# TinyMPC/TinyMPC

Hardware: AMD Instinct MI355X
Metric: QP solves/sec (+ ADMM iters/sec), 64k-batch quadrotor hover (higher is better)
Workload: dtype f64; 1 GPU; quadrotor_hovering (nx=12, nu=4, N=10), 65536 identical instances per GPU, closed-loop MPC steps from a cold start (BASELINE configs[1]); batch_per_gpu=65536, total_batch=65536, parallelism=batch-sharded x1, mpc_steps_per_launch=8, stats_exchange=none (one rank), launcher=plain process

## Files before the change

### tinympc_amd/csrc/admm_kernel.hip.h

```cpp
#pragma once
#include <hip/hip_runtime.h>
#include <stdint.h>

namespace tinympc_amd {

enum : int {
    TAB_MB = 0,
    TAB_MF1 = 256,
    TAB_MF2 = 512,
    TAB_PT = 768,
    TAB_VEC = 1024,
    TAB_BOUNDS = 1024 + 16 * 16,
};
enum : int {
    VEC_CB = 0,
    VEC_CF = 1,
    VEC_QR = 2,
    VEC_SMASK = 3,
    VEC_NIM = 4,
    VEC_SOCFLAG = 5,
    VEC_CONE_BASE = 6,
    VEC_CONE_MU = 7,
    VEC_LINFLAG = 9,
    VEC_TLINFLAG = 10,
// ... 549 lines not shown
    return __builtin_nontemporal_load(p);
#else
    return *p;
#endif
}
__device__ __forceinline__ void store_primal(double* p, double v) {
#if TINYMPC_PRIM_STORE == 1
    __builtin_nontemporal_store(v, p);
#elif TINYMPC_PRIM_STORE == 2
    asm volatile("global_store_dwordx2 %0, %1, off sc1" : : "v"(p), "v"(v) : "memory");
#elif TINYMPC_PRIM_STORE == 3
    asm volatile("global_store_dwordx2 %0, %1, off sc0 sc1" : : "v"(p), "v"(v) : "memory");
#elif TINYMPC_PRIM_STORE == 4
    asm volatile("global_store_dwordx2 %0, %1, off sc0 sc1 nt" : : "v"(p), "v"(v) : "memory");
#else
    *p = v;
#endif
}

__device__ __forceinline__ double grp_max16(double v) {
#pragma unroll
    for (int off = 8; off >= 1; off >>= 1) v = fmax(v, __shfl_xor(v, off, 16));
    return v;
}
template <int W>
__device__ __forceinline__ double grp_maxw(double v) {
#pragma unroll
    for (int off = W / 2; off >= 1; off >>= 1) v = fmax(v, __shfl_xor(v, off, W));
    return v;
}

__device__ __forceinline__ double soc_component(double s0, double s1, double s2, double mine, int c, float mu) {
#pragma clang fp contract(off)
    const double u0 = s2 * (double)mu;
    const double q0 = s0 * s0, q1 = s1 * s1;
    const double q = q0 + q1;
    const bool sure_inside = (u0 > 1e-30) && (q <= (u0 * u0) * (1.0 - 0x1p-20)) && (q < 1e70);
    if (__builtin_amdgcn_ballot_w64(!sure_inside) == 0ull) return mine;
    const float a = (float)sqrt(q);
    const double ad = (double)a;
    const bool below = ad <= -u0, inside = ad <= u0;
    const bool outside = !below && !inside && (ad >= fabs(u0));
    double r = (below || !inside) ? 0.0 : mine;
    if (__builtin_amdgcn_ballot_w64(outside) != 0ull) {
        const double scale = 0.5 * (1.0 + u0 / ad);
        const double last = (double)(a / mu);
        const double o = scale * ((c == 2) ? last : mine);
        r = outside ? o : r;
    }
    return r;
}

__device__ __forceinline__ bool soc_all_inside(double s0, double s1, double s2, float mu) {
#pragma clang fp contract(off)
    const double u0 = s2 * (double)mu;
    const double q0 = s0 * s0, q1 = s1 * s1;
    const double q = q0 + q1;
    const bool sure_inside = (u0 > 1e-30) & (u0 < 1e300) & (q <= (u0 * u0) * (1.0 - 0x1p-20)) & (q < 1e70);
    return __builtin_amdgcn_ballot_w64(!sure_inside) == 0ull;
}
__device__ __forceinline__ void soc_project3(double s0, double s1, double s2, float mu, float rmu, bool rmu_exact, double& r0, double& r1, double& r2) {
#pragma clang fp contract(off)
    const double u0 = s2 * (double)mu;
    const double q0 = s0 * s0, q1 = s1 * s1;
    const double q = q0 + q1;
    const float a = (float)sqrt(q);
    const double ad = (double)a;
    const bool below = ad <= -u0, inside = ad <= u0;
    const bool outside = !below && !inside && (ad >= fabs(u0));
    const bool zero = below || !inside;
    r0 = zero ? 0.0 : s0; r1 = zero ? 0.0 : s1; r2 = zero ? 0.0 : s2;
    if (__builtin_amdgcn_ballot_w64(outside) != 0ull) {
        const double scale = 0.5 * (1.0 + u0 / ad);
        const double last = (double)(rmu_exact ? a * rmu : a / mu);
        r0 = outside ? scale * s0 : r0;
        r1 = outside ? scale * s1 : r1;
        r2 = outside ? scale * last : r2;
    }
}
__device__ __forceinline__ int soc_items_of(unsigned heads, int nx, int n) {
    int c = 0;
    for (unsigned m = heads; m; m &= m - 1) c += (__builtin_ctz(m) < nx) ? n : n - 1;
    return c;
}
constexpr int soc_item_passes(int nx, int nu, int n) { return ((nx / 3) * n + (nu / 3) * (n - 1) + 15) / 16; }

constexpr int ADAPT_LOG = 32;
__device__ __forceinline__ double taylor_step(double a, double d, double b) {
#pragma clang fp contract(off)
    const double t = d * b;
    return a + t;
}

constexpr int solve_kernel_waves_per_simd(int nz, int n, bool soc, bool lin = false, bool adapt = false) {
    if (lin) return 1;
    if (adapt) return n <= 10 ? 2 : 1;
    return (n <= 10 || 2 * ((soc ? 8 : 6) * n + 2 * nz + 8) + 40 <= 256) ? 2 : 1;
}

#ifndef TINYMPC_LIN_WAVES
#define TINYMPC_LIN_WAVES 0
#endif
constexpr long solve_kernel_lin_lds(int nx, int nu, int n, bool soc, int lin, int kmax, bool ub) {
    const int nz = nx + nu, csl = (nz + 1) | 1, cs = (nz + 1) | 1;
    return 8L * (nx * 16 + (ub ? 2 : 2 * n * 16) + ((lin & 1) ? 3 * kmax * 16 + 2 * 4 * n * csl : 0) +
                 ((lin & 2) ? 3 * n * kmax * 16 + 2 * 4 * n * csl : 0) + (soc ? (4 * n + 1) * 3 * cs : 0));
}
constexpr bool solve_kernel_lin_planes(int nx, int nu, int n, bool soc, int lin, int kmax, bool ub) {
    return lin != 0 && solve_kernel_lin_lds(nx, nu, n, soc, lin, kmax, ub) <= 64 * 1024 - 512;
}
constexpr int solve_kernel_lin_waves(int nx, int nu, int n, bool soc, int lin, int kmax, bool ub) {
    if (!solve_kernel_lin_planes(nx, nu, n, soc, lin, kmax, ub)) return 1;
    if (TINYMPC_LIN_WAVES > 0) return TINYMPC_LIN_WAVES;
    return (solve_kernel_waves_per_simd(nx + nu, n, soc) == 2 && 8 * solve_kernel_lin_lds(nx, nu, n, soc, lin, kmax, ub) <= 158 * 1024) ? 2 : 1;
}
template <int NF, int KMAX_, int LW_, int LPI_>
__device__ __forceinline__ void project_halfspace_columns(const int t, const int inst, const int n, const int csl, const int R0, const int S0,
                                                          double* pv, double* pg, const double* tab, const int tab_stride, const int nk) {
#pragma clang fp contract(off)
    for (int c = S0 + t; c < n; c += LPI_) {
        const int at = (inst * n + c) * csl + R0;
        const double* tk = tab + c * tab_stride;
        double z[NF], t0[NF];
#pragma unroll
        for (int r = 0; r < NF; ++r) { z[r] = pv[at + r]; t0[r] = z[r]; }
        for (int k = 0; k < nk; ++k) {
            double cv = 0.0;
#pragma unroll
            for (int r = 0; r < NF; ++r) { const double pr = tk[k * LW_ + R0 + r] * z[r]; cv = cv + pr; }
            const double bk = tk[KMAX_ * LW_ + k * LW_ + R0];
            if (cv > bk) {
                const double dist = (cv - bk) / tk[2 * KMAX_ * LW_ + k * LW_ + R0];
#pragma unroll
                for (int r = 0; r < NF; ++r) { const double pr = dist * tk[k * LW_ + R0 + r]; z[r] = z[r] - pr; }
            }
        }
#pragma unroll
        for (int r = 0; r < NF; ++r) { pv[at + r] = z[r]; pg[at + r] = t0[r] - z[r]; }
    }
}

template <int NX, int NU, int N, bool SOC, bool DBG, int MODE, int LIN = 0, bool HET = false, int KMAX = LIN_KMAX, bool ADAPT = false, bool UB = false, bool HALF = false,
          bool PF = false>
__global__ __launch_bounds__(64)
__attribute__((amdgpu_waves_per_eu(LIN != 0 ? solve_kernel_lin_waves(NX, NU, N, SOC, LIN, KMAX, UB) : solve_kernel_waves_per_simd(NX + NU, N, SOC, false, ADAPT),
                                   LIN != 0 ? solve_kernel_lin_waves(NX, NU, N, SOC, LIN, KMAX, UB) : solve_kernel_waves_per_simd(NX + NU, N, SOC, false, ADAPT))))
void admm_solve_kernel(const SolveArgs P) {
    constexpr bool LS = (LIN & 1) != 0, LT = (LIN & 2) != 0;
    constexpr int NZ = NX + NU;
    static_assert(NZ <= 16, "one instance per 16-lane DPP row");
    constexpr bool FUSED = MODE == 2 && LIN == 0 && fused_shape(NX, NU);
    static_assert(!HALF || (NZ <= 8 && FUSED && !SOC && !DBG && !HET && !ADAPT), "half rows: nx+nu <= 8, the plain box kernel on its fused step blocks");
    static_assert(!PF || (MODE == 2 && !SOC && !DBG && LIN == 0 && !HET && !ADAPT), "prefetch form: the plain box kernel");
    constexpr int RL = HALF ? 8 : 16;
    constexpr int IPW = 64 / RL;
    constexpr int RECD = N * NZ;
    constexpr int PF_PIECES = (IPW * RECD * 8 + 1023) / 1024;
    constexpr int PF_ARR = PF_PIECES * 128;
    constexpr unsigned long long RMASK = HALF ? 0xFFull : 0xFFFFull;
    const int lane = threadIdx.x & 63;
    const int j = lane & (RL - 1);
    const int grp = lane / RL;
    const bool is_state = j < NX;
    const bool is_input = (j >= NX) && (j < NZ);

    __shared__ double sPt[NX * 16];
    __shared__ double sLo[UB ? 1 : N * 16];
    __shared__ double sHi[UB ? 1 : N * 16];
    __shared__ double sLin[LS ? 3 * KMAX * 16 : 1];
    __shared__ double sTLin[LT ? 3 * N * KMAX * 16 : 1];
#ifndef TINYMPC_SOC_PD
#define TINYMPC_SOC_PD 2
#endif
    constexpr int SPD = TINYMPC_SOC_PD, SPR = SPD + 1;
    constexpr int CS = SOC ? ((NZ + 1) | 1) : 1;
    constexpr int SLOT_D = 3 * CS;
    constexpr int PL_GC = CS, PL_VC = 2 * CS;
    __shared__ double sC[SOC ? (4 * N + 1) * SLOT_D : 1];
    __shared__ double sP[ADAPT ? 4 * NX * NX : 1];
    constexpr int AKC = NX > NU ? NX : NU;
    __shared__ double sTab[ADAPT ? 3 * 16 * AKC : 1];
    __shared__ double sDl[ADAPT ? 4 * ADAPT_LOG : 1];
    if constexpr (ADAPT)
        for (int e = lane; e < 3 * 16 * AKC; e += 64) {
            const int t = e / (16 * AKC), r = e % (16 * AKC);
            sTab[e] = P.atab[t * 256 + (r % AKC) * 16 + r / AKC];
        }
    if constexpr (LS) for (int e = lane; e < 3 * KMAX * 16; e += 64) sLin[e] = P.tab[TAB_BOUNDS + 2 * N * 16 + e];
    if constexpr (LT) for (int e = lane; e < 3 * N * KMAX * 16; e += 64) sTLin[e] = P.tab[TAB_BOUNDS + 2 * N * 16 + 3 * KMAX * 16 + e];
    for (int e = lane; e < NX * 16; e += 64) sPt[e] = P.tab[TAB_PT + e];
    for (int e = lane; e < N * 16; e += 64) {
        if constexpr (!UB) {
            sLo[e] = P.tab[TAB_BOUNDS + e];
            sHi[e] = P.tab[TAB_BOUNDS + N * 16 + e];
        }
    }
    double mb[NZ], mf1[NX], mf2[NU];
#pragma unroll
    for (int k = 0; k < NZ; ++k) mb[k] = P.tab[TAB_MB + k * 16 + j];
#pragma unroll
    for (int k = 0; k < NX; ++k) mf1[k] = P.tab[TAB_MF1 + k * 16 + j];
#pragma unroll
    for (int k = 0; k < NU; ++k) mf2[k] = P.tab[TAB_MF2 + (NX + k) * 16 + j];
    double cb = P.tab[TAB_VEC + VEC_CB * 16 + j];
    double cf = P.tab[TAB_VEC + VEC_CF * 16 + j];
    double qr = P.tab[TAB_VEC + VEC_QR * 16 + j];
    const double smask = P.tab[TAB_VEC + VEC_SMASK * 16 + j];
    const double nim = P.tab[TAB_VEC + VEC_NIM * 16 + j];
    bool soc_lane = false, proj_lane = false;
    int cone_base = -1, cone_c = 0;
    double socmask = 0.0;
    if constexpr (SOC) {
        socmask = P.tab[TAB_VEC + VEC_SOCFLAG * 16 + j];
        soc_lane = socmask != 0.0;
        cone_base = (int)P.tab[TAB_VEC + VEC_CONE_BASE * 16 + j];
        cone_c = (cone_base >= 0) ? (j - cone_base) : 0;
        proj_lane = soc_lane && cone_base >= 0;
    }
    constexpr int SOC_PASSES = SOC ? (soc_item_passes(NX, NU, N) > 0 ? soc_item_passes(NX, NU, N) : 1) : 1;
    int item_at[SOC_PASSES];
    float item_mu[SOC_PASSES], item_rmu[SOC_PASSES];
    bool mu_pow2 = true;
    int soc_passes = 0;
    if constexpr (SOC) {
        if (lane < 3) {
            sC[4 * N * SLOT_D + lane] = lane == 2 ? 1.0 : 0.0;
            sC[4 * N * SLOT_D + PL_GC + lane] = 0.0;
            sC[4 * N * SLOT_D + PL_VC + lane] = lane == 2 ? 1.0 : 0.0;
        }
        const unsigned heads = (unsigned)(__builtin_amdgcn_ballot_w64(proj_lane && cone_c == 0) & 0xFFFFull);
#pragma unroll
        for (int p = 0; p < SOC_PASSES; ++p) {
            int t = p * 16 + j;
            item_at[p] = 4 * N * SLOT_D; item_mu[p] = 1.0f;
            if (heads && p * 16 < soc_items_of(heads, NX, N)) soc_passes = p + 1;
            for (unsigned m = heads; m; m &= m - 1) {
                const int hb = __builtin_ctz(m);
                const int cnt = hb < NX ? N : N - 1;
                if (t >= 0 && t < cnt) {
                    item_at[p] = (grp * N + t + (hb < NX ? 0 : 1)) * SLOT_D + hb;
                    item_mu[p] = (float)P.tab[TAB_VEC + VEC_CONE_MU * 16 + hb];
                    t = -1;
                } else if (t >= 0) t -= cnt;
            }
            item_rmu[p] = 1.0f / item_mu[p];
            const unsigned mb_ = __float_as_uint(item_mu[p]);
            const bool p2 = (mb_ & 0x807FFFFFu) == 0u && (mb_ >> 23) >= 127u - 60u && (mb_ >> 23) <= 127u + 60u;
            if (__builtin_amdgcn_ballot_w64(!p2) != 0ull) mu_pow2 = false;
        }
    }
    bool lin_lane = false, tlin_lane = false;
    if constexpr (LS) lin_lane = P.tab[TAB_VEC + VEC_LINFLAG * 16 + j] != 0.0;
    if constexpr (LT) tlin_lane = P.tab[TAB_VEC + VEC_TLINFLAG * 16 + j] != 0.0;
    constexpr bool LPL = solve_kernel_lin_planes(NX, NU, N, SOC, LIN, KMAX, UB);
    constexpr bool LSP = LS && LPL, LTP = LT && LPL, LSR = LS && !LPL, LTR = LT && !LPL;
    constexpr int CSL = LPL ? ((NZ + 1) | 1) : 1;
    __shared__ double sLV[LSP ? 4 * N * CSL : 1], sLG[LSP ? 4 * N * CSL : 1];
    __shared__ double sTV[LTP ? 4 * N * CSL : 1], sTG[LTP ? 4 * N * CSL : 1];
    double ones[(LSR || LTR) ? 16 : 1];
#pragma unroll
    for (int k = 0; k < ((LSR || LTR) ? 16 : 1); ++k) ones[k] = 1.0;
    bool lin_x_on = false, lin_u_on = false, tlin_x_on = false, tlin_u_on = false;
    if constexpr (LS) { lin_x_on = P.tab[TAB_VEC + VEC_LINFLAG * 16] != 0.0; lin_u_on = P.tab[TAB_VEC + VEC_LINFLAG * 16 + NX] != 0.0; }
    if constexpr (LT) { tlin_x_on = P.tab[TAB_VEC + VEC_TLINFLAG * 16] != 0.0; tlin_u_on = P.tab[TAB_VEC + VEC_TLINFLAG * 16 + NX] != 0.0; }
    double rho = P.rho;
    __builtin_amdgcn_fence(__ATOMIC_RELEASE, "wavefront");
    __builtin_amdgcn_wave_barrier();

    const double lo_u = P.tab[TAB_BOUNDS + (N > 1 ? 16 : 0) + j], hi_u = P.tab[TAB_BOUNDS + N * 16 + (N > 1 ? 16 : 0) + j];
    const double lo_u0 = P.tab[TAB_BOUNDS + j], hi_u0 = P.tab[TAB_BOUNDS + N * 16 + j];
    const int ninst = PF ? P.batch : (P.index ? *P.count : (P.perm ? P.perm_count : P.batch));
    const int ntiles = (ninst + IPW - 1) / IPW;
    const bool resumed = !PF && P.index != nullptr;
    const bool has_traj = !PF && P.traj != nullptr;
    extern __shared__ __attribute__((aligned(16))) double sPF[];
    typedef const __attribute__((address_space(1))) void* pf_gptr;
    typedef __attribute__((address_space(3))) void* pf_lptr;
    constexpr int PF_S0 = 128, PF_S1 = PF_S0 + PF_ARR, PF_S2 = PF_S1 + PF_ARR, PF_S3 = PF_S2 + PF_ARR;
    auto pf_issue = [&](const int t) {
        const int tl = P.reverse ? ntiles - 1 - t : t;
        __builtin_amdgcn_global_load_lds((pf_gptr)(P.x0 + ((size_t)tl * (IPW * NX) + (size_t)lane * 2)), (pf_lptr)sPF, 16, 0, 0);
        const size_t t0 = (size_t)tl * (IPW * RECD) + (size_t)lane * 2;
        auto arr = [&](const double* p, const int at) {
#pragma unroll
            for (int q = 0; q < PF_PIECES; ++q) __builtin_amdgcn_global_load_lds((pf_gptr)(p + t0 + q * 128), (pf_lptr)(sPF + at + q * 128), 16, 0, 0);
        };
        if (!P.cold) { arr(P.slack, PF_S0); arr(P.dual, PF_S1); arr(P.slack_prev, PF_S2); }
        if (P.pf_mask & 8) arr(P.ref, P.cold ? PF_S0 : PF_S3);
    };
    unsigned pf_ticket = 0u;
    const int pf_shard = PF ? (int)(blockIdx.x % (unsigned)(P.pf_shards > 0 ? P.pf_shards : 1)) : 0;
    typedef __attribute__((address_space(1))) unsigned* pf_ctr_t;
    unsigned long long pf_ctr_bits = PF ? (unsigned long long)(P.pf_counter + 16 * pf_shard) : 0ull;
    if constexpr (PF) asm volatile("" : "+v"(pf_ctr_bits));
    const pf_ctr_t pf_ctr = (pf_ctr_t)pf_ctr_bits;
    auto pf_draw = [&]() { return lane == 0 ? __hip_atomic_fetch_add(pf_ctr, 1u, __ATOMIC_RELAXED, __HIP_MEMORY_SCOPE_AGENT) : 0u; };
    const unsigned pf_base = PF ? P.pf_base[pf_shard] : 0u;
    int pf_next = 0, pf_i = 0;
    bool pf_first = true;
    double* const sQX = sPF + PF_S3;
    if constexpr (PF) {
        if ((int)blockIdx.x < ntiles) {
            pf_issue((int)blockIdx.x);
            if (P.pf_static <= 1) pf_ticket = pf_draw();
        }
        if (P.ref_shared) {
            double rl = 0.0, qxs[N];
#pragma unroll
            for (int s = 0; s < N; ++s) {
                const bool valid = is_state || (is_input && s >= 1);
                const double r = valid ? P.ref[j - (is_input ? NZ : 0) + s * NZ] : 0.0;
                qxs[s] = -(r * qr);
                if (s == N - 1) rl = r;
            }
            double pt[NX];
#pragma unroll
            for (int k = 0; k < NX; ++k) pt[k] = sPt[k * 16 + j];
            double xp = 0.0;
            if constexpr (HALF) ring1_half<0, NX>(xp, rl, pt);
// ... 37 lines not shown
                for (int s = 0; s < N; ++s) {
                    const bool valid = is_state || (is_input && s >= 1);
                    const double r = valid ? sPF[at + lrow + s * NZ] : 0.0;
                    pfQXs[s] = -(r * qr);
                    if (s == N - 1) pf_rl = r;
                }
            };
            if (m & 8) { if (warm_t) own_ref(PF_S3); else own_ref(PF_S0); }
            else {
#pragma unroll
                for (int s = 0; s < N; ++s) pfQXs[s] = sQX[s * 16 + j];
            }
            if (warm_t) {
#pragma unroll
                for (int s = 0; s < N; ++s) pfVP[s] = sPF[PF_S2 + lrow + s * NZ];
            }
            asm volatile("s_waitcnt lgkmcnt(0)" ::: "memory");
            if (pf_next < ntiles) {
                if (pf_i + 2 >= P.pf_static) {
                    asm volatile("" ::: "memory");
                    pf_ticket = pf_draw();
                }
                pf_issue(pf_next);
            }
            ++pf_i;
        }
        (void)pfVN; (void)pfG; (void)pfVP; (void)pf_rl; (void)pf_x0; (void)pfQXs; (void)pf_first; (void)pf_ticket; (void)sQX; (void)pf_ctr; (void)pf_base; (void)pf_draw; (void)pf_i;
        if (slot < ninst) {
            const int b = PF ? slot : (resumed ? P.index[slot] : (P.perm ? P.perm[slot] : slot));
            const double* het = nullptr;
            if constexpr (HET) {
                het = P.het_tabs + (size_t)b * TAB_BOUNDS;
#pragma unroll
                for (int k = 0; k < NZ; ++k) mb[k] = het[TAB_MB + k * 16 + j];
#pragma unroll
                for (int k = 0; k < NX; ++k) mf1[k] = het[TAB_MF1 + k * 16 + j];
#pragma unroll
                for (int k = 0; k < NU; ++k) mf2[k] = het[TAB_MF2 + (NX + k) * 16 + j];
                cb = het[TAB_VEC + VEC_CB * 16 + j];
                cf = het[TAB_VEC + VEC_CF * 16 + j];
                qr = het[TAB_VEC + VEC_QR * 16 + j];
                rho = het[TAB_VEC + 8 * 16 + j];
            }
            if constexpr (ADAPT) {
                rho = P.arho[b];
                const double* aK = P.aK + (size_t)b * (NU * NX);
                if (is_state) {
#pragma unroll
                    for (int k = 0; k < NU; ++k) mb[NX + k] = -aK[k + NU * j];
#pragma unroll
                    for (int k = 0; k < NX; ++k) sP[grp * NX * NX + k + NX * j] = P.aP[(size_t)b * (NX * NX) + k + NX * j];
                } else if (is_input) {
#pragma unroll
                    for (int k = 0; k < NX; ++k) mf1[k] = -aK[(j - NX) + NU * k];
                }
                __builtin_amdgcn_fence(__ATOMIC_RELEASE, "wavefront");
                __builtin_amdgcn_wave_barrier();
            }
            const size_t lbase = (size_t)b * (N * NZ) + j - (is_input ? NZ : 0);
            double X[N], G[N], VN[N], VP[N], QX[N], Dn[N - 1];
            const int cw = grp * N * SLOT_D + (j < NZ ? j : NZ);
            const double x0v_in = is_state ? (PF ? pf_x0 : P.x0[(size_t)b * NX + j]) : 0.0;
            const int cl = grp * N * CSL + (j < NZ ? j : NZ);
            double VL[LSR ? N : 1], GL[LSR ? N : 1], VT[LTR ? N : 1], GT[LTR ? N : 1];
            double Qd[DBG ? N : 1], Pd[DBG ? N : 1], Dd[DBG ? N : 1];
            double ref_last = 0.0, qx_last_plain = 0.0;
#pragma unroll
            for (int s = 0; s < N; ++s) {
                const bool valid = is_state || (is_input && s >= 1);
                const size_t off = lbase + s * NZ;
                const bool warm = valid && !P.cold;
                if constexpr (PF) {
                    VN[s] = warm ? pfVN[s] : 0.0;
                    G[s] = warm ? pfG[s] : 0.0;
                    VP[s] = warm ? pfVP[s] : 0.0;
                    QX[s] = pfQXs[s];
                    X[s] = 0.0;
                    if (s == N - 1) ref_last = pf_rl;
                    continue;
                }
                const double r = valid ? (P.ref_shared ? P.ref[off - (size_t)b * (N * NZ)] : load_ref(P.ref + off)) : 0.0;
                VN[s] = warm ? P.slack[off] : 0.0;
                G[s] = warm ? P.dual[off] : 0.0;
                VP[s] = warm ? P.slack_prev[off] : 0.0;
                QX[s] = -(r * qr);
                X[s] = 0.0;
                if (s == N - 1) ref_last = r;
                if constexpr (SOC) {
                    double vc0 = (warm && soc_lane) ? (resumed ? P.cslack : P.prim)[off] : 0.0;
                    const double gc0 = (warm && soc_lane) ? P.cdual[off] : 0.0;
                    if (s == 0 && is_state && soc_lane && !resumed) vc0 = x0v_in;
                    sC[cw + s * SLOT_D] = vc0 - gc0;
                    sC[cw + s * SLOT_D + PL_GC] = gc0;
                    sC[cw + s * SLOT_D + PL_VC] = vc0;
                }
                if constexpr (LS) {
                    const double vl0 = (warm && lin_lane) ? (resumed ? P.lslack : P.prim)[off] : 0.0;
                    const double gl0 = (warm && lin_lane) ? P.ldual[off] : 0.0;
                    if constexpr (LSP) { sLV[cl + s * CSL] = vl0; sLG[cl + s * CSL] = gl0; } else { VL[s] = vl0; GL[s] = gl0; }
                }
                if constexpr (LT) {
                    const double vt0 = (warm && tlin_lane) ? (resumed ? P.tlslack : P.prim)[off] : 0.0;
                    const double gt0 = (warm && tlin_lane) ? P.tldual[off] : 0.0;
                    if constexpr (LTP) { sTV[cl + s * CSL] = vt0; sTG[cl + s * CSL] = gt0; } else { VT[s] = vt0; GT[s] = gt0; }
                }
                if constexpr (DBG) { Qd[s] = 0.0; Pd[s] = 0.0; Dd[s] = 0.0; }
            }
            double x0v = x0v_in;
            auto terminal_term = [&]() {
                double pt[NX];
#pragma unroll
                for (int k = 0; k < NX; ++k)
                    pt[k] = ADAPT ? sP[grp * NX * NX + k + NX * (is_state ? j : 0)] : (HET ? het[TAB_PT + k * 16 + j] : sPt[k * 16 + j]);
                double xp = 0.0;
                if constexpr (HALF) ring1_half<0, NX>(xp, ref_last, pt);
                else xp = ring_sum<MODE, 0, NX>(0.0, ref_last, pt);
                qx_last_plain = QX[N - 1];
                QX[N - 1] = is_state ? -xp : QX[N - 1];
            };
            int ndl = 0;
            auto flush_c = [&](int n) {
                __builtin_amdgcn_fence(__ATOMIC_RELEASE, "wavefront");
                __builtin_amdgcn_wave_barrier();
                if (P.aC2 && is_state) {
                    double* c2 = P.aC2 + (size_t)b * (NX * NX) + NX * j;
                    double v[NX], d[NX];
#pragma unroll
                    for (int k = 0; k < NX; ++k) { v[k] = c2[k]; d[k] = P.atab[ATAB_DC2 + k * 16 + j]; }
                    for (int i = 0; i < n; ++i) {
                        const double dl = sDl[grp * ADAPT_LOG + i];
#pragma unroll
                        for (int k = 0; k < NX; ++k) v[k] = taylor_step(v[k], dl, d[k]);
                    }
#pragma unroll
                    for (int k = 0; k < NX; ++k) c2[k] = v[k];
                }
                if (P.aC1 && j < NU) {
                    double* c1 = P.aC1 + (size_t)b * (NU * NU) + NU * j;
                    double v[NU], d[NU];
#pragma unroll
                    for (int k = 0; k < NU; ++k) { v[k] = c1[k]; d[k] = P.atab[ATAB_DC1 + k * 16 + j]; }
                    for (int i = 0; i < n; ++i) {
                        const double dl = sDl[grp * ADAPT_LOG + i];
#pragma unroll
                        for (int k = 0; k < NU; ++k) v[k] = taylor_step(v[k], dl, d[k]);
                    }
#pragma unroll
                    for (int k = 0; k < NU; ++k) c1[k] = v[k];
                }
            };
            if (!has_traj && !(PF && P.ref_shared)) terminal_term();
            const int traj_k0 = has_traj ? (P.traj_step0 + (P.traj_offsets ? P.traj_offsets[b] : 0)) : 0;

            int iter = 0, solved = 0, checked = 0;
            unsigned acc_iter = 0, acc_solved = 0;
            bool vp_touched = false;
            double rp = 0.0, rd = 0.0;
            const int nsteps = PF ? 1 : (P.steps > 1 ? P.steps : 1);
            const int iter_first = resumed ? P.iter_base : 0;
            for (int step = 0; step < nsteps; ++step) {
                X[0] = x0v;
                if (has_traj) {
                    if (is_state) {
#pragma unroll
                        for (int s = 0; s < N; ++s) {
                            int kk = traj_k0 + step + s;
                            kk = kk < P.traj_points ? kk : P.traj_points - 1;
                            const double r = P.traj[(size_t)kk * NX + j];
                            QX[s] = -(r * qr);
                            if (s == N - 1) ref_last = r;
                        }
                    }
                    terminal_term();
                }
                if (P.reset_duals) {
#pragma unroll
                    for (int s = 0; s < N; ++s) G[s] = 0.0;
                }
                if constexpr (SOC) {
                    if (step > 0) {
#pragma unroll
                        for (int s = 0; s < N; ++s) {
                            const double vc0 = soc_lane ? X[s] : 0.0;
                            sC[cw + s * SLOT_D] = vc0 - sC[cw + s * SLOT_D + PL_GC];
                            sC[cw + s * SLOT_D + PL_VC] = vc0;
                        }
                    }
                }
                if constexpr (LS) {
                    if (step > 0) {
#pragma unroll
                        for (int s = 0; s < N; ++s) { if constexpr (LSP) sLV[cl + s * CSL] = lin_lane ? X[s] : 0.0; else VL[s] = lin_lane ? X[s] : 0.0; }
                    } else if (is_state && lin_lane && !resumed) { if constexpr (LSP) sLV[cl] = x0v; else VL[0] = x0v; }
                }
                if constexpr (LT) {
                    if (step > 0) {
#pragma unroll
                        for (int s = 0; s < N; ++s) { if constexpr (LTP) sTV[cl + s * CSL] = tlin_lane ? X[s] : 0.0; else VT[s] = tlin_lane ? X[s] : 0.0; }
                    } else if (is_state && tlin_lane && !resumed) { if constexpr (LTP) sTV[cl] = x0v; else VT[0] = x0v; }
                }
                if constexpr (LPL) __builtin_amdgcn_fence(__ATOMIC_RELEASE, "wavefront");
                const int iter0 = iter_first;
                iter = iter0; solved = 0;
                if (resumed && P.check_termination > 0) checked = 1;
                int countdown = P.check_termination;
                double wr[SOC ? SPR : 1];
                bool gcz[SOC_PASSES];
#pragma unroll
                for (int p = 0; p < SOC_PASSES; ++p) gcz[p] = false;
                if constexpr (SOC) {
#pragma unroll
                    for (int d = 1; d <= SPR && d <= N; ++d) wr[(N - d) % SPR] = sC[cw + (N - d) * SLOT_D];
                }
                for (int it = iter0; it < P.max_iter; ++it) {
                    double lvr[LSP ? SPR : 1], lgr[LSP ? SPR : 1], tvr[LTP ? SPR : 1], tgr[LTP ? SPR : 1];
                    if constexpr (LPL) {
#pragma unroll
                        for (int d = 1; d <= SPR && d <= N; ++d) {
                            if constexpr (LSP) { lvr[(N - d) % SPR] = sLV[cl + (N - d) * CSL]; lgr[(N - d) % SPR] = sLG[cl + (N - d) * CSL]; }
                            if constexpr (LTP) { tvr[(N - d) % SPR] = sTV[cl + (N - d) * CSL]; tgr[(N - d) % SPR] = sTG[cl + (N - d) * CSL]; }
                        }
                    }
                    auto lin_w = [&](const int s_) { if constexpr (LSP) return lvr[s_ % SPR] - lgr[s_ % SPR]; else return VL[LSR ? s_ : 0] - GL[LSR ? s_ : 0]; };
                    auto tlin_w = [&](const int s_) { if constexpr (LTP) return tvr[s_ % SPR] - tgr[s_ % SPR]; else return VT[LTR ? s_ : 0] - GT[LTR ? s_ : 0]; };
                    double qhi;
                    {
                        double t = fma(-rho, VN[N - 1] - G[N - 1], QX[N - 1]);
                        if constexpr (SOC) t = fma(-rho, wr[(N - 1) % SPR], t);
                        if constexpr (LS) t = fma(-rho, lin_w(N - 1), t);
                        if constexpr (LT) t = fma(-rho, tlin_w(N - 1), t);
                        qhi = t;
                        if constexpr (DBG) {
                            double ql = fma(-rho, VN[N - 1] - G[N - 1], qx_last_plain);
                            if constexpr (SOC) ql = fma(-rho, wr[(N - 1) % SPR], ql);
                            if constexpr (LS) ql = fma(-rho, lin_w(N - 1), ql);
                            if constexpr (LT) ql = fma(-rho, tlin_w(N - 1), ql);
                            Qd[N - 1] = is_state ? ql : t;
                            Pd[N - 1] = t;
                        }
                    }
                    double pcur = qhi;
                    if constexpr (HALF) {
                        double tmpv = VN[N - 2] - G[N - 2];
#pragma unroll
                        for (int i = N - 2; i >= 0; --i) {
                            double qlo, res, dnp, tmpn;
                            constexpr int dummy = 0;
                            const int in = i > 0 ? i - 1 : dummy;
                            fused_backward_step_half<NX, NU>(qlo, res, dnp, tmpn, tmpv, VN[in], G[in], QX[i], rho, smask, cb, nim, cf, pcur, qhi, mb, mb + NX);
                            if (i + 1 <= N - 2) Dn[i + 1] = dnp;
                            tmpv = tmpn;
                            pcur = res;
                            qhi = qlo;
                        }
                        Dn[0] = fma(pcur, nim, cf);
                    }
#pragma unroll
                    for (int i = N - 2; i >= 0 && !HALF; --i) {
                        if constexpr (SOC) {
                            if (i >= SPD) wr[(i - SPD) % SPR] = sC[cw + (i - SPD) * SLOT_D];
                        }
                        if constexpr (LSP) { if (i >= SPD) { lvr[(i - SPD) % SPR] = sLV[cl + (i - SPD) * CSL]; lgr[(i - SPD) % SPR] = sLG[cl + (i - SPD) * CSL]; } }
                        if constexpr (LTP) { if (i >= SPD) { tvr[(i - SPD) % SPR] = sTV[cl + (i - SPD) * CSL]; tgr[(i - SPD) % SPR] = sTG[cl + (i - SPD) * CSL]; } }
                        if constexpr (SOC || LPL) __builtin_amdgcn_sched_barrier(0);
                        if constexpr (FUSED) {
                            double qlo, res;
                            if constexpr (SOC) fused_backward_step_soc<NX, NU>(qlo, res, VN[i], G[i], QX[i], wr[i % SPR], rho, smask, cb, pcur, qhi, mb, mb + NX);
                            else fused_backward_step<NX, NU>(qlo, res, VN[i], G[i], QX[i], rho, smask, cb, pcur, qhi, mb, mb + NX);
                            pcur = res;
                            Dn[i] = fma(res, nim, cf);
                            if constexpr (DBG) { Qd[i] = qlo; Pd[i] = res; Dd[i + 1] = res; }
                            qhi = qlo;
                            continue;
                        }
                        double qlo = fma(-rho, VN[i] - G[i], QX[i]);
                        if constexpr (SOC) qlo = fma(-rho, wr[i % SPR], qlo);
                        if constexpr (LS) qlo = fma(-rho, lin_w(i), qlo);
                        if constexpr (LT) qlo = fma(-rho, tlin_w(i), qlo);
                        const double res = ring_sum2<MODE, NX, NU>(fma(qlo, smask, cb), pcur, mb, qhi, mb + NX);
                        pcur = res;
                        Dn[i] = fma(res, nim, cf);
                        if constexpr (DBG) { Qd[i] = qlo; Pd[i] = res; Dd[i + 1] = res; }
                        qhi = qlo;
                    }
                    constexpr bool LAZY_RES = N <= 12;
                    constexpr bool TIGHT = FUSED && !HALF && LAZY_RES && !SOC && NX % 4 == 0;
                    double pmax = 0.0, dmax = 0.0;
                    auto slot_update = [&](const int s, const double lo, const double hi, const double gcv, const double glv, const double gtv) {
                        const double xi = X[s];
                        const double t = xi + G[s];
                        const double vn = TIGHT ? vclamp64(lo, hi, t) : vmin64(hi, vmax64(lo, t));
                        if constexpr (!LAZY_RES) {
                            pmax = resid_max<true>(pmax, xi - vn);
                            dmax = resid_max<true>(dmax, VP[s] - vn);
                        }
                        G[s] = t - vn;
                        VN[s] = vn;
                        if constexpr (SOC) {
                            sC[cw + s * SLOT_D] = fma(xi, socmask, gcv);
                        }
                        if constexpr (LSP) sLV[cl + s * CSL] = (lin_lane && (is_state || s >= 1)) ? (xi + glv) : 0.0;
                        if constexpr (LTP) sTV[cl + s * CSL] = (tlin_lane && (is_state || s >= 1)) ? (xi + gtv) : 0.0;
                        if constexpr (LSR || LTR) {
                            auto halfspaces = [&](double z, const double* tabk, const int nk) {
                                for (int k = 0; k < nk; ++k) {
                                    const double a = tabk[k * 16 + j];
                                    const double bk = tabk[KMAX * 16 + k * 16 + j];
                                    const double nn = tabk[2 * KMAX * 16 + k * 16 + j];
                                    const double prod = a * z;
                                    double cs = 0.0, ci = 0.0;
                                    ring1<0, NX>(cs, prod, ones);
                                    ring1<NX, NU>(ci, prod, ones);
                                    const double cv = is_state ? cs : ci;
                                    if (cv > bk) z = z - ((cv - bk) / nn) * a;
                                }
                                return z;
                            };
                            if constexpr (LSR) {
                                const bool on = lin_lane && (is_state || s >= 1);
                                double vl = on ? (xi + GL[s]) : 0.0;
                                vl = halfspaces(vl, sLin, P.n_lin);
                                GL[s] = on ? ((GL[s] + xi) - vl) : 0.0;
                                VL[s] = on ? vl : 0.0;
                            }
                            if constexpr (LTR) {
                                const bool on = tlin_lane && (is_state || s >= 1);
                                double vt = on ? (xi + GT[s]) : 0.0;
                                vt = halfspaces(vt, sTLin + s * 3 * KMAX * 16, P.n_tlin);
                                GT[s] = on ? ((GT[s] + xi) - vt) : 0.0;
                                VT[s] = on ? vt : 0.0;
                            }
                        }
                    };
                    double lo_c = UB ? lo_u0 : sLo[j], hi_c = UB ? hi_u0 : sHi[j];
                    double gr[SOC ? SPR : 1];
                    if constexpr (SOC) {
#pragma unroll
                        for (int d = 0; d < SPD && d < N; ++d) gr[d % SPR] = sC[cw + d * SLOT_D + PL_GC];
                    } else gr[0] = 0.0;
                    double glr[LSP ? SPR : 1], gtr[LTP ? SPR : 1];
                    glr[0] = 0.0; gtr[0] = 0.0;
                    if constexpr (LPL) {
#pragma unroll
                        for (int d = 0; d < SPD && d < N; ++d) {
                            if constexpr (LSP) glr[d % SPR] = sLG[cl + d * CSL];
                            if constexpr (LTP) gtr[d % SPR] = sTG[cl + d * CSL];
                        }
                    }
                    double tt_d = 0.0, vn_d = 0.0;
#pragma unroll
                    for (int i = 0; i < N - 1; ++i) {
                        const double lo_n = UB ? lo_u : sLo[(i + 1) * 16 + j], hi_n = UB ? hi_u : sHi[(i + 1) * 16 + j];
                        if constexpr (SOC) { if (i + SPD < N) gr[(i + SPD) % SPR] = sC[cw + (i + SPD) * SLOT_D + PL_GC]; }
                        if constexpr (LSP) { if (i + SPD < N) glr[(i + SPD) % SPR] = sLG[cl + (i + SPD) * CSL]; }
                        if constexpr (LTP) { if (i + SPD < N) gtr[(i + SPD) % SPR] = sTG[cl + (i + SPD) * CSL]; }
                        __builtin_amdgcn_sched_barrier(0);
                        if constexpr (FUSED) {
                            double tt, vn, xn, t = Dn[i];
                            const double xi = X[i];
                            if constexpr (HALF) {
                                double gnew;
                                fused_forward_step_half<NX, NU>(tt, vn, t, xn, gnew, xi, G[i], lo_c, hi_c, mf1, mf2);
                                X[i + 1] = xn;
                                if constexpr (!LAZY_RES) {
                                    pmax = resid_max<true>(pmax, xi - vn);
                                    dmax = resid_max<true>(dmax, VP[i] - vn);
                                }
                                G[i] = gnew;
                                VN[i] = vn;
                                lo_c = lo_n; hi_c = hi_n;
                                continue;
                            }
                            fused_forward_step<NX, NU, TIGHT>(tt, vn, t, xn, xi, G[i], lo_c, hi_c, mf1, mf2);
                            X[i + 1] = xn;
                            if constexpr (!LAZY_RES) {
                                pmax = resid_max<true>(pmax, xi - vn);
                                dmax = resid_max<true>(dmax, VP[i] - vn);
                            }
                            if constexpr (TIGHT) {
                                __builtin_amdgcn_sched_barrier(0);
                                if (i > 0) G[i - 1] = pinned_sub64(tt_d, vn_d);
                                tt_d = tt; vn_d = vn;
                            } else G[i] = tt - vn;
                            VN[i] = vn;
                            if constexpr (SOC) sC[cw + i * SLOT_D] = fma(xi, socmask, gr[i % SPR]);
                            lo_c = lo_n; hi_c = hi_n;
                            continue;
                        }
                        const double t = ring_sum<MODE, 0, NX>(Dn[i], X[i], mf1);
                        X[i + 1] = ring_short<MODE, NX, NU>(t, t, mf2);
                        slot_update(i, lo_c, hi_c, gr[SOC ? i % SPR : 0], glr[LSP ? i % SPR : 0], gtr[LTP ? i % SPR : 0]);
                        lo_c = lo_n; hi_c = hi_n;
                    }
                    if constexpr (TIGHT && N >= 2) G[N - 2] = tt_d - vn_d;
                    (void)tt_d; (void)vn_d;
                    slot_update(N - 1, lo_c, hi_c, gr[SOC ? (N - 1) % SPR : 0], glr[LSP ? (N - 1) % SPR : 0], gtr[LTP ? (N - 1) % SPR : 0]);
                    if constexpr (LPL) {
                        __builtin_amdgcn_fence(__ATOMIC_RELEASE, "wavefront");
                        __builtin_amdgcn_wave_barrier();
                        if constexpr (LSP) {
                            if (lin_x_on) project_halfspace_columns<NX, KMAX, 16, 16>(j, grp, N, CSL, 0, 0, sLV, sLG, sLin, 0, P.n_lin);
                            if (lin_u_on) project_halfspace_columns<NU, KMAX, 16, 16>(j, grp, N, CSL, NX, 1, sLV, sLG, sLin, 0, P.n_lin);
                        }
                        if constexpr (LTP) {
                            if (tlin_x_on) project_halfspace_columns<NX, KMAX, 16, 16>(j, grp, N, CSL, 0, 0, sTV, sTG, sTLin, 3 * KMAX * 16, P.n_tlin);
                            if (tlin_u_on) project_halfspace_columns<NU, KMAX, 16, 16>(j, grp, N, CSL, NX, 1, sTV, sTG, sTLin, 3 * KMAX * 16, P.n_tlin);
                        }
                        __builtin_amdgcn_fence(__ATOMIC_RELEASE, "wavefront");
                        __builtin_amdgcn_wave_barrier();
                    }
                    bool conv = false;
                    auto termination = [&]() {
                        if (countdown > 0 && --countdown == 0) {
                            countdown = P.check_termination;
                            checked = 1;
                            constexpr int PS0 = N >= 2 ? 1 : 0, PS1 = N - 1;
                            auto lost = [&](const int s) {
                                return (int)(fabs(X[s] - VN[s]) >= P.tol_pri) | (int)(fabs(VP[s] - VN[s]) * rho >= P.tol_dua);
                            };
                            const bool maybe = ((int)!(rho > 0.0) | (int)!(lost(PS0) | lost(PS1))) != 0;
                            unsigned long long fold = __ballot(maybe);
                            fold &= fold >> 1; fold &= fold >> 2; fold &= fold >> 4;
                            if constexpr (!HALF) fold &= fold >> 8;
                            const bool any_row = (fold & (HALF ? 0x0101010101010101ull : 0x0001000100010001ull)) != 0ull;
                            const bool last_test = (P.max_iter - 1 - it) < P.check_termination;
                            if (last_test || any_row) {
                                if constexpr (LAZY_RES) {
#pragma unroll
                                    for (int s = 0; s < N; ++s) {
                                        pmax = resid_max<false>(pmax, X[s] - VN[s]);
                                        dmax = resid_max<false>(dmax, VP[s] - VN[s]);
                                    }
                                }
                                rp = pmax;
                                rd = dmax * rho;
                                const bool ok = (rp < P.tol_pri) && (rd < P.tol_dua);
                                const unsigned long long bal = __ballot(ok);
                                conv = ((bal >> (grp * RL)) & RMASK) == RMASK;
                            }
                        }
                    };
                    if constexpr (SOC) {
                        __builtin_amdgcn_fence(__ATOMIC_RELEASE, "wavefront");
                        __builtin_amdgcn_wave_barrier();
                        double n0 = sC[item_at[0]], n1 = sC[item_at[0] + 1], n2 = sC[item_at[0] + 2];
#pragma unroll
                        for (int d = 1; d <= SPR && d <= N; ++d) wr[(N - d) % SPR] = sC[cw + (N - d) * SLOT_D];
                        termination();
                        bool any_exact = false;
#pragma unroll
                        for (int p = 0; p < SOC_PASSES; ++p) {
                            if (p > 0 && p >= soc_passes) break;
                            const int at = item_at[p];
                            if (p > 0) { n0 = sC[at]; n1 = sC[at + 1]; n2 = sC[at + 2]; }
                            const double s0 = n0, s1 = n1, s2 = n2;
                            if (soc_all_inside(s0, s1, s2, item_mu[p])) {
                                sC[at + PL_VC] = s0; sC[at + PL_VC + 1] = s1; sC[at + PL_VC + 2] = s2;
                                if (!gcz[p]) {
                                    sC[at + PL_GC] = 0.0; sC[at + PL_GC + 1] = 0.0; sC[at + PL_GC + 2] = 0.0;
                                    gcz[p] = true;
                                }
                            } else {
                                double r0, r1, r2;
                                soc_project3(s0, s1, s2, item_mu[p], item_rmu[p], mu_pow2, r0, r1, r2);
                                const double g0 = s0 - r0, g1 = s1 - r1, g2 = s2 - r2;
                                sC[at + PL_VC] = r0; sC[at + PL_VC + 1] = r1; sC[at + PL_VC + 2] = r2;
                                sC[at + PL_GC] = g0; sC[at + PL_GC + 1] = g1; sC[at + PL_GC + 2] = g2;
                                sC[at] = r0 - g0; sC[at + 1] = r1 - g1; sC[at + 2] = r2 - g2;
                                gcz[p] = false;
                                any_exact = true;
                            }
                        }
                        if (it == iter0 && !proj_lane) {
#pragma unroll
                            for (int s = 0; s < N; ++s) sC[cw + s * SLOT_D + PL_GC] = 0.0;
                        }
                        __builtin_amdgcn_fence(__ATOMIC_RELEASE, "wavefront");
                        __builtin_amdgcn_wave_barrier();
                        if (any_exact) {
#pragma unroll
                            for (int d = 1; d <= SPR && d <= N; ++d) wr[(N - d) % SPR] = sC[cw + (N - d) * SLOT_D];
                        }
                    }
                    iter += 1;
                    if constexpr (ADAPT) {
                        if (it > 0 && it % 5 == 0) {
                            double at[NX];
#pragma unroll
                            for (int k = 0; k < NX; ++k) at[k] = sTab[j * AKC + k];
                            double pri_res = 0.0, ax_max = 0.0, z_max = 0.0, dual_res = 0.0, px_max = 0.0, aty_max = 0.0, q_max = 0.0;
                            double pxq_max = 0.0;
#pragma unroll
                            for (int i = 0; i < N - 1; ++i) {
                                const double axs = ring_sum<MODE, 0, NX>(0.0, X[i], mf1);
                                const double dyn = ring_short<MODE, NX, NU>(axs, is_input ? X[i + 1] : 0.0, mf2) - X[i + 1];
                                const double a = is_state ? dyn : X[i + 1];
                                const double zz = VN[i + 1];
                                const bool on = is_state || is_input;
                                pri_res = fmax(pri_res, on ? fabs(a - zz) : 0.0);
                                ax_max = fmax(ax_max, on ? fabs(a) : 0.0);
                                z_max = fmax(z_max, on ? fabs(zz) : 0.0);
                                const double init = is_state ? (i >= 1 ? -G[i] : 0.0) : G[i + 1];
                                const double aty = ring_sum<MODE, 0, NX>(init, G[i + 1], at);
                                const double xs = is_state ? X[i] : X[i + 1];
                                const double px = qr * xs;
                                dual_res = fmax(dual_res, on ? fabs((px + px) + aty) : 0.0);
                                pxq_max = fmax(pxq_max, on ? fabs(px) : 0.0);
                                aty_max = fmax(aty_max, on ? fabs(aty) : 0.0);
                            }
                            {
                                double prow[NX];
#pragma unroll
                                for (int k = 0; k < NX; ++k) prow[k] = sP[grp * NX * NX + (is_state ? j : 0) + NX * k];
                                const double pxl = ring_sum<MODE, 0, NX>(0.0, X[N - 1], prow);
                                const double ql = qr * X[N - 1];
                                const double atyl = -G[N - 1];
                                dual_res = fmax(dual_res, is_state ? fabs((pxl + ql) + atyl) : 0.0);
                                px_max = fmax(pxq_max, is_state ? fabs(pxl) : 0.0);
                                aty_max = fmax(aty_max, is_state ? fabs(atyl) : 0.0);
                                q_max = fmax(pxq_max, is_state ? fabs(ql) : 0.0);
                            }
                            pri_res = grp_max16(pri_res); ax_max = grp_max16(ax_max); z_max = grp_max16(z_max);
                            dual_res = grp_max16(dual_res); px_max = grp_max16(px_max); aty_max = grp_max16(aty_max); q_max = grp_max16(q_max);
                            const double pri_norm = fmax(ax_max, z_max);
                            const double dual_norm = fmax(fmax(px_max, aty_max), q_max);
                            const double eps = 1e-10;
                            const double normalized_pri = pri_res / (pri_norm + eps);
                            const double normalized_dual = dual_res / (dual_norm + eps);
                            const double ratio = normalized_pri / (normalized_dual + eps);
                            double new_rho = rho * sqrt(ratio);
                            if (P.aclip) new_rho = fmin(fmax(new_rho, P.arho_min), P.arho_max);
                            const double delta = new_rho - rho;
                            if (is_state) {
#pragma unroll
                                for (int k = 0; k < NU; ++k) mb[NX + k] = -taylor_step(-mb[NX + k], delta, sTab[(16 + j) * AKC + k]);
#pragma unroll
                                for (int k = 0; k < NX; ++k) {
                                    const int e = grp * NX * NX + k + NX * j;
                                    sP[e] = taylor_step(sP[e], delta, sTab[(32 + j) * AKC + k]);
                                }
                            } else if (is_input) {
#pragma unroll
                                for (int k = 0; k < NX; ++k) mf1[k] = -taylor_step(-mf1[k], delta, sTab[(16 + j) * AKC + k]);
                            }
                            if (P.aC1 || P.aC2) {
                                if (j == 0) sDl[grp * ADAPT_LOG + ndl] = delta;
                                if (++ndl == ADAPT_LOG) { flush_c(ndl); ndl = 0; }
                            }
                            rho = new_rho;
                            __builtin_amdgcn_fence(__ATOMIC_RELEASE, "wavefront");
                            __builtin_amdgcn_wave_barrier();
                            QX[N - 1] = qx_last_plain;
                            terminal_term();
                        }
                    }
                    if constexpr (!SOC) termination();
                    if (conv) { solved = 1; break; }
#pragma unroll
                    for (int s = 0; s < N; ++s) VP[s] = VN[s];
                    vp_touched = true;
                }
                acc_iter += (unsigned)(iter - iter0);
                acc_solved += (unsigned)solved;
                if (P.iter_log && j == 0) P.iter_log[(size_t)step * P.batch + b] = solved ? iter : -iter;
                if (P.u0_log && is_input) P.u0_log[((size_t)step * P.batch + b) * NU + (j - NX)] = X[1];
                if (nsteps > 1) {
                    x0v = is_state ? X[1] : 0.0;
                }
            }

            constexpr bool FLS = TINYMPC_FULL_LINE_STORES != 0 && (PF || TINYMPC_FULL_LINE_STORES == 2) && !SOC && LIN == 0 && !DBG;
            if (FLS && (P.store_mask & 32) == 0) {
                if constexpr (FLS) {
                    const size_t seg = (size_t)b * (N * NZ) + j;
                    const bool in_row = j < NZ;
#pragma unroll
                    for (int s = 0; s < N; ++s) {
                        const size_t off = seg + s * NZ;
                        const double xs = is_input ? (s + 1 < N ? X[s + 1 < N ? s + 1 : s] : 0.0) : X[s];
                        const double vs = is_input ? (s + 1 < N ? VN[s + 1 < N ? s + 1 : s] : 0.0) : VN[s];
                        const double gs = is_input ? (s + 1 < N ? G[s + 1 < N ? s + 1 : s] : 0.0) : G[s];
                        const double ps = is_input ? (s + 1 < N ? VP[s + 1 < N ? s + 1 : s] : 0.0) : VP[s];
                        if (in_row) {
                            if (P.store_mask & 1) {
                                if (acc_iter > 0) { if constexpr (PF) P.prim[off] = xs; else store_primal(P.prim + off, xs); }
                                else if (s == 0 && is_state) P.prim[off] = xs;
                            }
                            if (P.store_mask & 2) P.slack[off] = vs;
                            if (P.store_mask & 4) P.dual[off] = gs;
                            if ((P.store_mask & 8) && vp_touched) P.slack_prev[off] = ps;
                        }
                    }
                }
            } else
#pragma unroll
            for (int s = 0; s < N; ++s) {
                const bool valid = is_state || (is_input && s >= 1);
                const size_t off = lbase + s * NZ;
                if (valid) {
                    if (((P.store_mask & 1) || ((P.store_mask & 32) && s <= 1)) && (acc_iter > 0 || (s == 0 && is_state))) {
                        if constexpr (SOC || LIN != 0) P.prim[off] = X[s];
                        else store_primal(P.prim + off, X[s]);
                    }
                    if (P.store_mask & 2) P.slack[off] = VN[s];
                    if (P.store_mask & 4) P.dual[off] = G[s];
                    if ((P.store_mask & 8) && vp_touched) P.slack_prev[off] = VP[s];
                    if constexpr (SOC) {
                        if (soc_lane && (P.store_mask & 16)) {
                            P.cslack[off] = sC[cw + s * SLOT_D + ((proj_lane || iter <= iter_first) ? PL_VC : 0)];
                            P.cdual[off] = sC[cw + s * SLOT_D + PL_GC];
                        }
                    }
                    if constexpr (LSP) { if (lin_lane && (P.store_mask & 16)) { P.lslack[off] = sLV[cl + s * CSL]; P.ldual[off] = sLG[cl + s * CSL]; } }
                    if constexpr (LTP) { if (tlin_lane && (P.store_mask & 16)) { P.tlslack[off] = sTV[cl + s * CSL]; P.tldual[off] = sTG[cl + s * CSL]; } }
                    if constexpr (LSR) { if (lin_lane && (P.store_mask & 16)) { P.lslack[off] = VL[s]; P.ldual[off] = GL[s]; } }
                    if constexpr (LTR) { if (tlin_lane && (P.store_mask & 16)) { P.tlslack[off] = VT[s]; P.tldual[off] = GT[s]; } }
                    if constexpr (DBG) {
                        if (P.dbg_qr && acc_iter > 0) {
                            P.dbg_qr[off] = Qd[s];
                            P.dbg_pd[off] = is_state ? Pd[s] : Dd[s];
                        }
                    }
                }
            }
            if constexpr (ADAPT) {
                if (ndl > 0) flush_c(ndl);
                if (j == 0) P.arho[b] = rho;
                if (is_state) {
#pragma unroll
                    for (int k = 0; k < NU; ++k) P.aK[(size_t)b * (NU * NX) + k + NU * j] = -mb[NX + k];
#pragma unroll
                    for (int k = 0; k < NX; ++k) P.aP[(size_t)b * (NX * NX) + k + NX * j] = sP[grp * NX * NX + k + NX * j];
                }
            }
            if (P.x0_next && acc_iter > 0 && is_state) P.x0_next[(size_t)b * NX + j] = X[1];
            const double ps = grp_maxw<RL>(is_state ? rp : 0.0), pi = grp_maxw<RL>(is_input ? rp : 0.0);
            const double ds = grp_maxw<RL>(is_state ? rd : 0.0), di = grp_maxw<RL>(is_input ? rd : 0.0);
            if (P.next_index) {
                const bool open = j == 0 && !solved;
                const unsigned long long m = __ballot(open);
                if (m) {
                    const int first = __ffsll((long long)m) - 1;
                    int at = 0;
                    if (lane == first) at = atomicAdd(P.next_count, __popcll(m));
                    at = __shfl(at, first);
                    if (open) P.next_index[at + __popcll(m & ((1ull << lane) - 1ull))] = b;
                }
            }
            if (j == 0) {
                P.status[b] = make_int4(iter, solved, solved ? 1 : 11, checked);
                double4 rr = make_double4(ps, pi, ds, di);
                *reinterpret_cast<double4*>(P.resid + (size_t)b * 4) = rr;
                if (P.accum) {
                    if constexpr (PF) {
                        __hip_atomic_fetch_add(&P.accum[b].x, acc_iter, __ATOMIC_RELAXED, __HIP_MEMORY_SCOPE_AGENT);
                        __hip_atomic_fetch_add(&P.accum[b].y, acc_solved, __ATOMIC_RELAXED, __HIP_MEMORY_SCOPE_AGENT);
                    } else {
                        uint2 ac = P.accum[b];
                        ac.x += acc_iter;
                        ac.y += acc_solved;
                        P.accum[b] = ac;
                    }
                }
            }
        }
    }
}

}
```

Before: 2.890 billion QP solves/s.

## Run ADMM iteration loop with scalar wave-uniform control and LDS-backed previous slack

For the fused short-horizon box kernel, the ADMM iteration loop becomes an inner do-while whose counters, termination countdown and convergence pre-check run in scalar registers via inline SALU assembly and wave ballots. Previous-slack vectors VP move to an LDS double buffer swapped by pointer arithmetic, which avoids per-iteration register copies and lowers register pressure. The full residual check only runs when the cheap two-slot ballot test passes. It adds fragile inline asm, extra LDS traffic per iteration and more complex exit bookkeeping.

```diff
diff --git a/tinympc_amd/csrc/admm_kernel.hip.h b/tinympc_amd/csrc/admm_kernel.hip.h
--- a/tinympc_amd/csrc/admm_kernel.hip.h
+++ b/tinympc_amd/csrc/admm_kernel.hip.h
@@ -725,6 +725,9 @@
     constexpr bool FUSED = MODE == 2 && LIN == 0 && fused_shape(NX, NU);
     static_assert(!HALF || (NZ <= 8 && FUSED && !SOC && !DBG && !HET && !ADAPT), "half rows: nx+nu <= 8, the plain box kernel on its fused step blocks");
     static_assert(!PF || (MODE == 2 && !SOC && !DBG && LIN == 0 && !HET && !ADAPT), "prefetch form: the plain box kernel");
+    constexpr bool ULOOP = FUSED && !HALF && N <= 12 && !SOC && NX % 4 == 0 && !ADAPT && LIN == 0 && !DBG && !PF && !HET;
+    constexpr int PS0 = N >= 2 ? 1 : 0, PS1 = N - 1;
+    constexpr int VPBUF = N * 64 * 8;
     constexpr int RL = HALF ? 8 : 16;
     constexpr int IPW = 64 / RL;
     constexpr int RECD = N * NZ;
@@ -738,6 +741,7 @@
     const bool is_input = (j >= NX) && (j < NZ);
 
     __shared__ double sPt[NX * 16];
+    __shared__ double sVP[ULOOP ? 2 * N * 64 : 1];
     __shared__ double sLo[UB ? 1 : N * 16];
     __shared__ double sHi[UB ? 1 : N * 16];
     __shared__ double sLin[LS ? 3 * KMAX * 16 : 1];
@@ -1081,6 +1085,15 @@
             if (!has_traj && !(PF && P.ref_shared)) terminal_term();
             const int traj_k0 = has_traj ? (P.traj_step0 + (P.traj_offsets ? P.traj_offsets[b] : 0)) : 0;
 
+            int vpb = lane * 8;
+            auto vp_cell = [&](const int boff, const int s) -> double& {
+                return *reinterpret_cast<double*>(reinterpret_cast<char*>(sVP) + boff + s * 512);
+            };
+            if constexpr (ULOOP) {
+#pragma unroll
+                for (int s = 0; s < N; ++s) vp_cell(vpb, s) = VP[s];
+            }
+            (void)vpb; (void)vp_cell;
             int iter = 0, solved = 0, checked = 0;
             unsigned acc_iter = 0, acc_solved = 0;
             bool vp_touched = false;
@@ -1141,7 +1154,23 @@
 #pragma unroll
                     for (int d = 1; d <= SPR && d <= N; ++d) wr[(N - d) % SPR] = sC[cw + (N - d) * SLOT_D];
                 }
-                for (int it = iter0; it < P.max_iter; ++it) {
+                unsigned cd = (unsigned)P.check_termination;
+                const int full_from = rho > 0.0 ? P.max_iter - P.check_termination : -2147483647 - 1;
+                double rho_v = rho;
+                int vpk = 2 * lane * 8 + VPBUF;
+                if constexpr (ULOOP) asm volatile("" : "+v"(rho_v), "+v"(vpk));
+                (void)cd; (void)full_from; (void)rho_v; (void)vpk;
+                for (int it = iter0; it < P.max_iter; it += ULOOP ? 0 : 1) {
+                  int why = 0;
+                  bool conv = false;
+                  const int it_in = it;
+                  const unsigned cd_in = cd;
+                  (void)why; (void)it_in; (void)cd_in;
+                  do {
+                    if constexpr (ULOOP) {
+                        VP[PS0] = vp_cell(vpb, PS0);
+                        VP[PS1] = vp_cell(vpb, PS1);
+                    }
                     double lvr[LSP ? SPR : 1], lgr[LSP ? SPR : 1], tvr[LTP ? SPR : 1], tgr[LTP ? SPR : 1];
                     if constexpr (LPL) {
 #pragma unroll
@@ -1195,7 +1224,7 @@
                         if constexpr (FUSED) {
                             double qlo, res;
                             if constexpr (SOC) fused_backward_step_soc<NX, NU>(qlo, res, VN[i], G[i], QX[i], wr[i % SPR], rho, smask, cb, pcur, qhi, mb, mb + NX);
-                            else fused_backward_step<NX, NU>(qlo, res, VN[i], G[i], QX[i], rho, smask, cb, pcur, qhi, mb, mb + NX);
+                            else fused_backward_step<NX, NU>(qlo, res, VN[i], G[i], QX[i], ULOOP ? rho_v : rho, smask, cb, pcur, qhi, mb, mb + NX);
                             pcur = res;
                             Dn[i] = fma(res, nim, cf);
                             if constexpr (DBG) { Qd[i] = qlo; Pd[i] = res; Dd[i + 1] = res; }
@@ -1214,6 +1243,7 @@
                     }
                     constexpr bool LAZY_RES = N <= 12;
                     constexpr bool TIGHT = FUSED && !HALF && LAZY_RES && !SOC && NX % 4 == 0;
+                    static_assert(!ULOOP || TIGHT, "the wave-uniform loop is a form of the short box loop");
                     double pmax = 0.0, dmax = 0.0;
                     auto slot_update = [&](const int s, const double lo, const double hi, const double gcv, const double glv, const double gtv) {
                         const double xi = X[s];
@@ -1338,12 +1368,10 @@
                         __builtin_amdgcn_fence(__ATOMIC_RELEASE, "wavefront");
                         __builtin_amdgcn_wave_barrier();
                     }
-                    bool conv = false;
                     auto termination = [&]() {
                         if (countdown > 0 && --countdown == 0) {
                             countdown = P.check_termination;
                             checked = 1;
-                            constexpr int PS0 = N >= 2 ? 1 : 0, PS1 = N - 1;
                             auto lost = [&](const int s) {
                                 return (int)(fabs(X[s] - VN[s]) >= P.tol_pri) | (int)(fabs(VP[s] - VN[s]) * rho >= P.tol_dua);
                             };
@@ -1411,7 +1439,7 @@
                             for (int d = 1; d <= SPR && d <= N; ++d) wr[(N - d) % SPR] = sC[cw + (N - d) * SLOT_D];
                         }
                     }
-                    iter += 1;
+                    if constexpr (!ULOOP) iter += 1;
                     if constexpr (ADAPT) {
                         if (it > 0 && it % 5 == 0) {
                             double at[NX];
@@ -1483,7 +1511,68 @@
                             terminal_term();
                         }
                     }
+                    if constexpr (ULOOP) {
+                        (void)termination; (void)conv;
+                        const bool lp = fmax(fabs(X[PS0] - VN[PS0]), fabs(X[PS1] - VN[PS1])) >= P.tol_pri;
+                        const bool ld = fmax(fabs(VP[PS0] - VN[PS0]), fabs(VP[PS1] - VN[PS1])) * rho >= P.tol_dua;
+                        const unsigned long long x = __builtin_amdgcn_ballot_w64(lp) | __builtin_amdgcn_ballot_w64(ld) | ~__builtin_amdgcn_ballot_w64(true);
+                        asm("v_sub_u32 %0, %1, %0" : "+v"(vpb) : "v"(vpk));
+#pragma unroll
+                        for (int s = 0; s < N; ++s) vp_cell(vpb, s) = VN[s];
+                        unsigned xlo = (unsigned)x, t0, t1;
+                        asm volatile("s_add_i32 %[it], %[it], 1\n\t"
+                                     "s_add_u32 %[cd], %[cd], -1\n\t"
+                                     "s_cmp_lg_u32 %[cd], 0\n\t"
+                                     "s_cbranch_scc1 1f\n\t"
+                                     "s_mov_b32 %[cd], %[ct]\n\t"
+                                     "s_cmp_gt_i32 %[it], %[ff]\n\t"
+                                     "s_cselect_b32 %[xlo], 0, %[xlo]\n\t"
+                                     "s_sub_u32 %[t0], %[xlo], 0x10001\n\t"
+                                     "s_sub_u32 %[t1], %[xhi], 0x10001\n\t"
+                                     "s_andn2_b32 %[t0], %[t0], %[xlo]\n\t"
+                                     "s_andn2_b32 %[t1], %[t1], %[xhi]\n\t"
+                                     "s_or_b32 %[t0], %[t0], %[t1]\n\t"
+                                     "s_and_b32 %[t0], %[t0], 0x80008000\n\t"
+                                     "s_cselect_b32 %[why], 1, 0\n\t"
+                                     "s_cbranch_scc1 2f\n"
+                                     "1:\n\t"
+                                     "s_cmp_ge_i32 %[it], %[mx]\n\t"
+                                     "s_cselect_b32 %[why], 2, 0\n"
+                                     "2:"
+                                     : [it] "+s"(it), [cd] "+s"(cd), [xlo] "+s"(xlo), [why] "=&s"(why), [t0] "=&s"(t0), [t1] "=&s"(t1)
+                                     : [xhi] "s"((unsigned)(x >> 32)), [ct] "s"(P.check_termination), [ff] "s"(full_from), [mx] "s"(P.max_iter)
+                                     : "scc");
+                        continue;
+                    }
                     if constexpr (!SOC) termination();
+                  } while (ULOOP && why == 0);
+                    if constexpr (ULOOP) {
+                        iter = it;
+                        if (P.check_termination > 0 && cd_in <= (unsigned)(it - it_in)) checked = 1;
+                        if (it - it_in > 1) vp_touched = true;
+                        if (why == 1) {
+                            double pmax = 0.0, dmax = 0.0;
+                            asm volatile("" ::: "memory");
+#pragma unroll
+                            for (int s = 0; s < N; ++s) if (s != PS0 && s != PS1) VP[s] = vp_cell(vpk - vpb, s);
+#pragma unroll
+                            for (int s = 0; s < N; ++s) {
+                                pmax = resid_max<false>(pmax, X[s] - VN[s]);
+                                dmax = resid_max<false>(dmax, VP[s] - VN[s]);
+                            }
+                            rp = pmax;
+                            rd = dmax * rho;
+                            const bool ok = (rp < P.tol_pri) && (rd < P.tol_dua);
+                            const unsigned long long bal = __ballot(ok);
+                            if (((bal >> (grp * RL)) & RMASK) == RMASK) {
+                                solved = 1;
+                                vpb = vpk - vpb;
+                                break;
+                            }
+                        }
+                        vp_touched = true;
+                        continue;
+                    }
                     if (conv) { solved = 1; break; }
 #pragma unroll
                     for (int s = 0; s < N; ++s) VP[s] = VN[s];
@@ -1498,6 +1587,11 @@
                 }
             }
 
+            if constexpr (ULOOP) {
+                asm volatile("" ::: "memory");
+#pragma unroll
+                for (int s = 0; s < N; ++s) VP[s] = vp_cell(vpb, s);
+            }
             constexpr bool FLS = TINYMPC_FULL_LINE_STORES != 0 && (PF || TINYMPC_FULL_LINE_STORES == 2) && !SOC && LIN == 0 && !DBG;
             if (FLS && (P.store_mask & 32) == 0) {
                 if constexpr (FLS) {
```

Result: slower. 2.755 billion QP solves/s (-4.6%).
